# xingchensong/TouchNet

Hardware: AMD Instinct MI355X
Metric: audio+text tokens/sec/node (packed seq, full train step) + step MFU (higher is better)
Workload: dtype bf16

## Files before the change

### touchnet_amd/bin/train.py

```python
from __future__ import annotations

import os

from dataclasses import dataclass
from typing import Optional

import torch
import torch.distributed as dist

from touchnet_amd.utils.distributed import ParallelDims, dist_sum
from touchnet_amd.utils.optimizer import FusedAdamW, linear_warmup_linear_decay
from touchnet_amd.utils.train_spec import TrainSpec, get_train_spec


@dataclass
class TrainConfig:
    training_model_name: str = "llama_mi355"
    training_seed: int = 2025
    training_max_norm: float = 1.0
    training_mixed_precision_param: str = "bfloat16"
    training_mixed_precision_reduce: str = "float32"
    training_fsdp_reshard_after_forward: str = "never"
    training_tp_sequence_parallel: bool = True
    training_enable_loss_parallel: bool = False
# ... 86 lines not shown
                                enable_loss_parallel=job.training_enable_loss_parallel)
            if sharded and n == 1:
                dims = _ForceShard(dims)
            view = {"dp_shard_cp": fsdp_mesh}
            if tp > 1:
                view["tp"] = self.tp_mesh
            import dataclasses
            model = self.spec.parallelize_fn(model, _MeshView(view), dims,
                                             dataclasses.replace(job, training_dp_engine="fsdp2"))
        if sharded:
            model.to_empty(device=device)
            with torch.no_grad():
                model.post_init()
                if self.spec.additional_post_init_fn:
                    self.spec.additional_post_init_fn(model, device)
        else:
            model.to_empty(device=device)
            with torch.no_grad():
                model.post_init()
                if self.spec.additional_post_init_fn:
                    self.spec.additional_post_init_fn(model, device)
            if device.type == "cuda":
                model.to(getattr(torch, job.training_mixed_precision_param))
        if tp > 1:
            from touchnet_amd.models.tensor_parallel import reinit_tp_shards
            seq_cfg = getattr(model_config, "text_config", model_config)
            reinit_tp_shards(model, job.training_seed, getattr(seq_cfg, "initializer_range", 0.02))
        self.model = model
        self.dp_engine = None
        if flat:
            from touchnet_amd.utils.zero_dp import FlatShardedDataParallel
            self.dp_engine = FlatShardedDataParallel(model, fsdp_mesh,
                                                     reduce_dtype=getattr(torch, job.training_mixed_precision_reduce))
        if optimizer_factory is not None:
            self.optimizer = optimizer_factory(self.dp_engine.named_shards() if flat else model.parameters())
        elif flat:
            self.optimizer = FusedAdamW(self.dp_engine.named_shards(), lr=job.lr_scheduler_lr,
                                        weight_decay=job.optimizer_weight_decay, max_norm=job.training_max_norm,
                                        process_group=fsdp_mesh.get_group())
        else:
            from touchnet_amd.models.tensor_parallel import tp_param_ids
            tp_group, tp_ids = tp_param_ids([model])
            self.optimizer = FusedAdamW(model.named_parameters(), lr=job.lr_scheduler_lr,
                                        weight_decay=job.optimizer_weight_decay, max_norm=job.training_max_norm,
                                        process_group=fsdp_mesh.get_group() if sharded else None,
                                        tp_group=tp_group, tp_param_ids=tp_ids)
            want = os.environ.get("TN_PIPELINE_OPTIMIZER")
            want = job.training_pipeline_optimizer if want is None else want == "1"
            if (want and device.type == "cuda" and not sharded
                    and not any(hasattr(p, "_local_tensor") for p in model.parameters())):
                from touchnet_amd.utils.optimizer import pipeline_updates_under_forward
                pipeline_updates_under_forward(model, self.optimizer)
        self.wgrad_queue = None
        if (device.type == "cuda" and not sharded and not flat and tp == 1 and not ac and self.cp_group is None
                and self.cp_emulate is None):
            import touchnet_amd.functional as _F
            layers = [ly for m in model.modules() if hasattr(m, "deferred_wgrad_layers") for ly in m.deferred_wgrad_layers()]
            if layers and _F.DEFERRED_WGRAD:
                self.wgrad_queue = _F.DeferredWgrad(layers)
                self.wgrad_queue.enabled = False
        self.step = 0
        self.dp_cp_group = fsdp_mesh.get_group() if fsdp_mesh is not None and shard_world > 1 else None

    def next_batch(self, batch: dict) -> dict:
        out = {}
        for k, v in batch.items():
            out[k] = v.to(self.device, non_blocking=True) if isinstance(v, torch.Tensor) else v
        ns = out["num_sentence"]
        ns = ns.to(self.device, torch.float32) if isinstance(ns, torch.Tensor) else torch.tensor(
            float(ns), dtype=torch.float32, device=self.device)
        out["num_sentence"] = dist_sum(ns.reshape(1), self.dp_group) if self.dp_world > 1 else ns.reshape(1)
        if self.cp_group is not None or self.cp_emulate is not None:
            from touchnet_amd.utils.context_parallel import ContextParallel
            T = out["labels"].shape[1]
            if self.cp is None or self.cp.T != T:
                self.cp = ContextParallel(self.cp_group, T, emulate=self.cp_emulate)
            if not isinstance(out.get("attention_mask"), torch.Tensor):
                out["attention_mask"] = torch.ones(out["labels"].shape[0], T, dtype=torch.int64, device=self.device)
            if self.job.training_cp_halo_exchange:
                src = batch.get("attention_mask")
                self.cp.set_documents(src if isinstance(src, torch.Tensor) else out["attention_mask"])
            else:
                self.cp.need = None
            presharded = out.pop("audio_cp_sharded", False)
            if isinstance(out.get("audio_positions"), torch.Tensor) and not presharded:
                self._shard_audio(batch, out)
            if "labelled_rows_max" in out:
                lab = batch.get("labels")
                if "labelled_rows_max_cp" in out:
                    out["labelled_rows_max"] = int(out.pop("labelled_rows_max_cp")[self.cp.rank])
                elif isinstance(lab, torch.Tensor) and not lab.is_cuda:
                    out["labelled_rows_max"] = int((self.cp.shard(lab, dim=1) != -100).sum())
                else:
                    out.pop("labelled_rows_max")
            for k in ("input_ids", "labels", "position_ids", "sentence_lens", "input_features", "inputs_embeds"):
                if isinstance(out.get(k), torch.Tensor) and not (k == "input_features" and "audio_rows" in out):
                    out[k] = self.cp.shard(out[k], dim=1)
            out.pop("valid_rows_max", None)
            out["context_parallel"] = self.cp
        return out

    def _shard_audio(self, batch: dict, out: dict) -> None:
        host = lambda k: (batch[k] if isinstance(batch.get(k), torch.Tensor) and not batch[k].is_cuda else out[k].cpu()).numpy()
        feats = out["input_features"]
        rows_per_clip = ((feats.shape[-1] - 1) // 2 + 1) // 2
        clips, pos, rows = self.cp.shard_audio(host("audio_positions"), host("audio_output_lengths"), rows_per_clip)
        dev = lambda a: torch.from_numpy(a).to(self.device, non_blocking=True)
        clips_d = dev(clips)
        out["input_features"] = feats.index_select(0, clips_d)
        out["audio_output_lengths"] = out["audio_output_lengths"].index_select(0, clips_d)
        out["audio_positions"], out["audio_rows"] = dev(pos), dev(rows)

    def forward_loss(self, data: dict):
        data = dict(data)
        labels, ns, sl = data.pop("labels"), data.pop("num_sentence"), data.pop("sentence_lens")
        data.pop("shift_labels", None)
        if self.job.training_enable_fused_ce:
            pred = self.model(**data, labels=labels, sentence_lens=sl, num_sentence=ns,
                              ce_chunk_tokens=self.job.training_ce_chunk_tokens,
                              ce_compact=self.job.training_ce_compact_rows)
            return pred.loss, pred.loss_per_token, pred.acc
        pred = self.model(**data)
        loss, per_token = self.spec.loss_fn(pred.logits, labels, sl, ns)
        acc = self.spec.acc_fn(pred.logits, labels) if self.spec.acc_fn else None
        return loss, per_token, acc

    def train_step(self, data: dict) -> dict:
        self.optimizer.zero_grad()
        if self.dp_engine is not None:
            self.dp_engine.zero_grad()
        loss, per_token, acc = self.forward_loss(data)
        if self.wgrad_queue is not None:
            self.wgrad_queue.enabled = True
            try:
                loss.backward()
                self.wgrad_queue.flush()
            finally:
                self.wgrad_queue.enabled = False
        else:
            loss.backward()
        from touchnet_amd.models.backend import ops as _ops
        if hasattr(_ops(), "sync_wgrad_stream"):
            _ops().sync_wgrad_stream()
        if self.tp_mesh is not None:
            from touchnet_amd.models.tensor_parallel import reduce_sequence_partial_grads
            reduce_sequence_partial_grads(self.model)
        if self.dp_engine is not None:
            self.dp_engine.finish_backward()
        lr = self.job.lr_scheduler_lr * linear_warmup_linear_decay(
            self.step, self.job.lr_scheduler_warmup_steps, self.job.lr_scheduler_steps)
        grad_norm = self.optimizer.step(lr)
        if self.dp_engine is not None:
            self.dp_engine.gather_params()
        self.step += 1
        return {"loss_per_sample": loss.detach(), "loss_per_token": per_token, "acc": acc, "grad_norm": grad_norm}

    def reduce_metrics(self, loss_per_sample, loss_per_token, acc=None):
        from touchnet_amd.utils.distributed import dist_max, dist_mean, dist_min
        g = self.dp_cp_group
        ls, lt = loss_per_sample.detach(), loss_per_token.detach()
        zero = torch.zeros((), device=ls.device)
        if g is None:
            a = acc.detach() if acc is not None else zero
            return (ls, lt, lt, a, a)
        return (dist_sum(ls, g), dist_mean(lt, g), dist_max(lt, g),
                dist_mean(acc.detach(), g) if acc is not None else zero,
                dist_min(acc.detach(), g) if acc is not None else zero)

    @torch.no_grad()
    def dev_step(self, data: dict):
        return self.reduce_metrics(*self.forward_loss(data))

    @torch.no_grad()
    def dev(self, batches) -> dict:
        was_training = self.model.training
        self.model.eval()
        if getattr(self.optimizer, "wait_updates", None):
            self.optimizer.wait_updates()
        try:
            metrics = [self.dev_step(self.next_batch(b)) for b in batches]
        finally:
            self.model.train(was_training)
        if not metrics:
            return {}
        col = lambda i: torch.stack([m[i].reshape(()) for m in metrics])
        return {"global_avg_loss_per_sample": col(0).mean(), "global_avg_loss_per_token": col(1).mean(),
                "global_max_loss_per_token": col(2).max(), "global_avg_acc": col(3).mean(),
                "global_min_acc": col(4).min(), "batches": len(metrics)}
```

### touchnet_amd/csrc/gemm_kernel.h

```cpp
#pragma once

#include <stdlib.h>

#include <type_traits>
#include <utility>
#include <vector>

#include "common.h"

namespace tn {
namespace gemm {

constexpr int BM = 256, BN = 256;
constexpr int SLOT = 32768;
constexpr int LDS_BYTES = 5 * SLOT;
constexpr int NT = 512;
constexpr int MAXSEG = 3;

typedef __attribute__((address_space(3))) void* lds_ptr_t;
typedef __attribute__((ext_vector_type(2))) uint32_t u32x2_t;
typedef __attribute__((ext_vector_type(4))) uint32_t u32x4_t;

struct Seg {
  const bf16_t* A;
  const bf16_t* B;
  long long lda, ldb;
  int K;
  int pad_;
};

struct Grp {
  bf16_t* C;
  long long ldc;
  int M, N, nbm, nbn;
  int start;
  int stages;
};

struct Rec {
  Seg seg;
  Grp grp;
  bf16_t* bias_out;
};
typedef const __attribute__((address_space(4))) Rec* rec_ptr_t;
constexpr int MAXTAB = 1024;
constexpr int TABCHUNK = 32;

constexpr int EPI_PLAIN = 0, EPI_GROUPED = 1, EPI_SWIGLU_FWD = 2, EPI_SWIGLU_BWD = 3, EPI_BIASG = 4, EPI_ROPE = 5;
constexpr int EPI_GELU_FWD = 6, EPI_GELU_BWD = 7, EPI_TABLE = 8;

struct Params {
  Seg seg[MAXSEG];
  int nseg;
  int M, N;
  bf16_t* C;
  bf16_t* Ct;
  const bf16_t* bias;
  long long ldc, ldct;
  int accumulate;
  const bf16_t* addend;
  long long ldadd;
  int nbm, nbn;
  int stages;
  int splitk, kchunk;
  float* ws;
  int tile0, ntiles;
  int c_f32;
  Grp grp[MAXSEG];
  int ngrp;
  bf16_t* C2;
  bf16_t* C3;
  const bf16_t* E1;
  const bf16_t* E2;
  long long lde;
  bf16_t* bias_out;
  float* bias_ws;
  const bf16_t* rope_cos;
  const bf16_t* rope_sin;
  int rope_d;
  const Rec* table;
};

__device__ __forceinline__ int xcd_chunk(int bid, int total) {
  const int xcd = bid & 7, local = bid >> 3;
  const int q = total >> 3, r = total & 7;
  return (xcd < r ? xcd * (q + 1) : r * (q + 1) + (xcd - r) * q) + local;
}

__device__ __forceinline__ void panel_group(int vid, int nbm, int nbn, int& tm, int& tn) {
  constexpr int GM = 8;
  const int per_group = GM * nbn;
  const int g = vid / per_group, w = vid - g * per_group;
  const int gm = min(GM, nbm - g * GM);
  tm = g * GM + w % gm;
  tn = w / gm;
}

__device__ __forceinline__ void tile_of_block(int bid, int nbm, int nbn, int& tm, int& tn) {
  panel_group(xcd_chunk(bid, nbm * nbn), nbm, nbn, tm, tn);
}

typedef f32x16_t Acc[4][2];
// ... 29 lines not shown
        const int row = wave * 32 + q * 8 + (lane >> 3);
        voff[q] = row * ld2 + (((lane & 7) ^ ((row >> 1) & 7)) << 4);
      }
    } else {
#pragma unroll
      for (int q = 0; q < 4; ++q) {
        const int k = wave * 8 + q * 2 + (lane >> 5);
        const int u = lane & 31;
        const int ch = M16 ? ((u & 3) ^ (((k >> 3) & 1) << 1)) : (u & 3);
        voff[q] = k * ld2 + ((((u >> 2) ^ (k & 3)) << 6) | (ch << 4));
      }
    }
  }

  __device__ __forceinline__ void open(const bf16_t* X, long long ld, int K, int R, int origin, int wave, int lane) {
    ld2 = (int)(ld * 2);
    if constexpr (!KMAJ) {
      const long long bytes = R > origin ? (long long)(R - origin - 1) * ld2 + 2LL * K : 0LL;
      rs = __builtin_amdgcn_make_buffer_rsrc((void*)(X + (long long)origin * ld), 0, (int)min(bytes, 0x7fffffffLL),
                                             0x00020000);
      step = 128;
    } else {
      const long long bytes = ((long long)(K - 1) * ld + (R - origin)) * 2;
      rs = __builtin_amdgcn_make_buffer_rsrc((void*)(X + origin), 0, (int)min(bytes, 0x7fffffffLL), 0x00020000);
      step = 64 * ld2;
    }
    set_voff(wave, lane);
    soff = 0;
    left = (K + 63) >> 6;
  }
  __device__ __forceinline__ void kill(const void* any) {
    rs = __builtin_amdgcn_make_buffer_rsrc((void*)any, 0, 0, 0x00020000);
    soff = 0;
    step = 0;
    left = 0x7fffffff;
  }
};

template <bool KMAJ, int NB>
struct Frags {
  bf16x8_t v[NB];
  u32x2_t h[KMAJ ? NB : 1][2];
};

template <int OFF>
__device__ __forceinline__ u32x2_t ds_tr16(uint32_t addr) {
  u32x2_t r;
  asm volatile("ds_read_b64_tr_b16 %0, %1 offset:%2" : "=v"(r) : "v"(addr), "n"(OFF));
  return r;
}

template <bool AK, bool BK, bool HAS_CT, bool SPLITK = false, bool OUT_F32 = false, int EPI = EPI_PLAIN>
struct Kernel {
  static_assert(EPI == EPI_PLAIN || EPI == EPI_GROUPED || EPI == EPI_BIASG || EPI == EPI_TABLE,
                "Kernel: plain / grouped / bias-gradient epilogues (the fused ones are Kernel16's)");
  static constexpr bool MULTI = EPI == EPI_GROUPED || EPI == EPI_TABLE;
  static constexpr bool BIASG = EPI == EPI_BIASG || EPI == EPI_TABLE;
  static_assert(!MULTI || (!HAS_CT && !SPLITK), "grouped launch: whole tiles, no transposed copy");
  static_assert(!BIASG || (AK && BK && !HAS_CT), "bias gradient: weight-gradient mode");
  struct Out {
    bf16_t* C;
    long long ldc;
    int M, N;
  };
  template <bool KMAJ, int NB>
  struct Reader {
    int x[4];
    __device__ __forceinline__ Reader(int lane, int row0 ) {
      const int l31 = lane & 31, hi = lane >> 5;
      if constexpr (!KMAJ) {
        const int f = (l31 >> 1) & 7;
#pragma unroll
        for (int q = 0; q < 4; ++q) x[q] = (row0 + l31) * 128 + (((2 * q + hi) ^ f) << 4);
      } else {
        const int s4 = lane & 15, j = s4 >> 2, w = s4 & 3, half = (lane >> 4) & 1;
#pragma unroll
        for (int b = 0; b < 4; ++b)
          x[b] = (8 * hi + j) * 512 + half * 32 + w * 8 + ((((row0 >> 5) + (b < NB ? b : 0)) ^ j) << 6);
      }
    }
    template <int Q, int B>
    __device__ __forceinline__ void read(const char* smem, int sbase, Frags<KMAJ, NB>& f) const {
      if constexpr (!KMAJ) {
        f.v[B] = __builtin_bit_cast(bf16x8_t, *reinterpret_cast<const u32x4_t*>(smem + sbase + x[Q] + B * 4096));
      } else {
        const uint32_t a = (uint32_t)(size_t)(lds_ptr_t)smem + (uint32_t)(sbase + x[B]);
        f.h[B][0] = ds_tr16<(16 * Q) * 512>(a);
        f.h[B][1] = ds_tr16<(16 * Q + 4) * 512>(a);
      }
    }
  };

  static __device__ __forceinline__ void wait_frags(Frags<AK, 4>& a, Frags<BK, 2>& b) {
    if constexpr (AK && BK) {
      asm volatile("s_waitcnt lgkmcnt(0)"
                   : "+v"(a.h[0][0]), "+v"(a.h[0][1]), "+v"(a.h[1][0]), "+v"(a.h[1][1]), "+v"(a.h[2][0]), "+v"(a.h[2][1]),
                     "+v"(a.h[3][0]), "+v"(a.h[3][1]), "+v"(b.h[0][0]), "+v"(b.h[0][1]), "+v"(b.h[1][0]), "+v"(b.h[1][1]));
    } else if constexpr (AK) {
      asm volatile("s_waitcnt lgkmcnt(0)"
                   : "+v"(a.h[0][0]), "+v"(a.h[0][1]), "+v"(a.h[1][0]), "+v"(a.h[1][1]), "+v"(a.h[2][0]), "+v"(a.h[2][1]),
                     "+v"(a.h[3][0]), "+v"(a.h[3][1]));
    } else if constexpr (BK) {
      asm volatile("s_waitcnt lgkmcnt(0)" : "+v"(b.h[0][0]), "+v"(b.h[0][1]), "+v"(b.h[1][0]), "+v"(b.h[1][1]));
    }
    if constexpr (AK) {
#pragma unroll
      for (int i = 0; i < 4; ++i) {
        const u32x4_t t = {a.h[i][0].x, a.h[i][0].y, a.h[i][1].x, a.h[i][1].y};
        a.v[i] = __builtin_bit_cast(bf16x8_t, t);
      }
    }
    if constexpr (BK) {
#pragma unroll
      for (int j = 0; j < 2; ++j) {
        const u32x4_t t = {b.h[j][0].x, b.h[j][0].y, b.h[j][1].x, b.h[j][1].y};
        b.v[j] = __builtin_bit_cast(bf16x8_t, t);
      }
    }
  }

  static __device__ __forceinline__ void run(const Params& p, char* smem) { body(p, smem); }

  static __device__ __forceinline__ void body(const Params& p, char* smem) {
    const int tid = threadIdx.x;
    int lane = tid & 63;
    const int wave = __builtin_amdgcn_readfirstlane(tid >> 6);
    const int wr = wave >> 2, wc = wave & 3;

    const int bid = blockIdx.x, G = gridDim.x;
    const int tiles = p.ntiles;
    const int mine = ((SPLITK ? tiles * p.splitk : tiles) - bid + G - 1) / G;
    const rec_ptr_t tab = (rec_ptr_t)p.table;
    auto seg_of = [&](int g) {
      if constexpr (EPI == EPI_TABLE) {
        Seg s;
        s.A = tab[g].seg.A;
        s.B = tab[g].seg.B;
        s.lda = tab[g].seg.lda;
        s.ldb = tab[g].seg.ldb;
        s.K = tab[g].seg.K;
        s.pad_ = 0;
        return s;
      } else {
        return p.seg[g];
      }
    };
    auto grp_of = [&](int g) {
      if constexpr (EPI == EPI_TABLE) {
        Grp r;
        r.C = tab[g].grp.C;
        r.ldc = tab[g].grp.ldc;
        r.M = tab[g].grp.M;
        r.N = tab[g].grp.N;
        r.nbm = tab[g].grp.nbm;
        r.nbn = tab[g].grp.nbn;
        r.start = tab[g].grp.start;
        r.stages = tab[g].grp.stages;
        return r;
      } else {
        return p.grp[g];
      }
    };
    auto origin_g = [&](int k, int& m0, int& n0, int& g) {
      int tm, tn, u = bid + k * G;
      if constexpr (SPLITK) u -= (u / tiles) * tiles;
      u += p.tile0;
      g = 0;
      if constexpr (EPI == EPI_TABLE) {
        u = xcd_chunk(u, tiles);
        int hi = p.ngrp - 1;
        while (g < hi) {
          const int mid = (g + hi + 1) >> 1;
          if (tab[mid].grp.start <= u) g = mid;
          else hi = mid - 1;
        }
      } else if constexpr (EPI == EPI_GROUPED) {
        if (p.ngrp > 1 && u >= p.grp[1].start) g = 1;
        if (p.ngrp > 2 && u >= p.grp[2].start) g = 2;
      }
      if constexpr (EPI == EPI_TABLE) {
        const Grp r = grp_of(g);
        panel_group(u - r.start, r.nbm, r.nbn, tm, tn);
      } else if constexpr (EPI == EPI_GROUPED) {
        const Grp r = grp_of(g);
        tile_of_block(u - r.start, r.nbm, r.nbn, tm, tn);
      } else {
        tile_of_block(u, p.nbm, p.nbn, tm, tn);
      }
      m0 = tm * BM;
      n0 = tn * BN;
    };
    auto origin = [&](int k, int& m0, int& n0) {
      int g;
      origin_g(k, m0, n0, g);
    };
    auto split_of = [&](int k) { return (bid + k * G) / tiles; };

    Stream<AK> sA;
    Stream<BK> sB;
    int ka = 0, kb = 0;
    auto open_a = [&](int s) {
      int m0, n0;
      origin(ka, m0, n0);
      if constexpr (SPLITK) {
        const int k0 = split_of(ka) * p.kchunk * 64, klen = min(p.seg[0].K - k0, p.kchunk * 64);
        if (klen > 0) sA.open(p.seg[0].A + (AK ? (long long)k0 * p.seg[0].lda : (long long)k0), p.seg[0].lda, klen, p.M,
                              m0, wave, lane);
        else sA.kill(p.C);
        sA.left = p.kchunk;
      } else if constexpr (MULTI) {
        int g;
        origin_g(ka, m0, n0, g);
        const Seg sg = seg_of(g);
        sA.open(sg.A, sg.lda, sg.K, grp_of(g).M, m0, wave, lane);
      } else {
        sA.open(p.seg[s].A, p.seg[s].lda, p.seg[s].K, p.M, m0, wave, lane);
      }
      sA.seg = s;
    };
    auto open_b = [&](int s) {
      int m0, n0;
      origin(kb, m0, n0);
      if constexpr (SPLITK) {
        const int k0 = split_of(kb) * p.kchunk * 64, klen = min(p.seg[0].K - k0, p.kchunk * 64);
        if (klen > 0) sB.open(p.seg[0].B + (BK ? (long long)k0 * p.seg[0].ldb : (long long)k0), p.seg[0].ldb, klen, p.N,
                              n0, wave, lane);
        else sB.kill(p.C);
        sB.left = p.kchunk;
      } else if constexpr (MULTI) {
        int g;
        origin_g(kb, m0, n0, g);
        const Seg sg = seg_of(g);
        sB.open(sg.B, sg.ldb, sg.K, grp_of(g).N, n0, wave, lane);
// ... 30 lines not shown
    open_b(0);

    Reader<AK, 4> ra(lane, wr * 128);
    Reader<BK, 2> rb(lane, wc * 64);

    Acc acc;
    auto zero_acc = [&]() {
#pragma unroll
      for (int i = 0; i < 4; ++i)
#pragma unroll
        for (int j = 0; j < 2; ++j)
#pragma unroll
          for (int r = 0; r < 16; ++r) acc[i][j][r] = 0.f;
    };
    zero_acc();

    Frags<AK, 4> ae, ao;
    Frags<BK, 2> be, bo;

#define TN_PIN() __builtin_amdgcn_sched_barrier(0)
    auto read_frag = [&](auto QC, auto FC, int sa, int sb, Frags<AK, 4>& a, Frags<BK, 2>& b) {
      constexpr int Q = decltype(QC)::value, F = decltype(FC)::value;
      if constexpr (F < 2) rb.template read<Q, F>(smem, sb * SLOT, b);
      else ra.template read<Q, F - 2>(smem, sa * SLOT, a);
    };
    auto read_all = [&](auto QC, int sa, int sb, Frags<AK, 4>& a, Frags<BK, 2>& b) {
      read_frag(QC, std::integral_constant<int, 0>{}, sa, sb, a, b);
      read_frag(QC, std::integral_constant<int, 1>{}, sa, sb, a, b);
      read_frag(QC, std::integral_constant<int, 2>{}, sa, sb, a, b);
      read_frag(QC, std::integral_constant<int, 3>{}, sa, sb, a, b);
      read_frag(QC, std::integral_constant<int, 4>{}, sa, sb, a, b);
      read_frag(QC, std::integral_constant<int, 5>{}, sa, sb, a, b);
    };
    auto mma = [&](const Frags<AK, 4>& a, const Frags<BK, 2>& b, int i, int j) {
      acc[i][j] = __builtin_amdgcn_mfma_f32_32x32x16_bf16(b.v[j], a.v[i], acc[i][j], 0, 0, 0);
    };

    float bsum = 0.f;
    bool bias_on = false;
    auto bias_accum = [&](const Frags<AK, 4>& a) {
      auto add = [&](const bf16x8_t& v) {
        const u32x4_t w = __builtin_bit_cast(u32x4_t, v);
        bsum += ((__uint_as_float(w.x << 16) + __uint_as_float(w.x & 0xffff0000u)) +
                 (__uint_as_float(w.y << 16) + __uint_as_float(w.y & 0xffff0000u))) +
                ((__uint_as_float(w.z << 16) + __uint_as_float(w.z & 0xffff0000u)) +
                 (__uint_as_float(w.w << 16) + __uint_as_float(w.w & 0xffff0000u)));
      };
      if (wc == 0) add(a.v[0]);
      else if (wc == 1) add(a.v[1]);
      else if (wc == 2) add(a.v[2]);
      else add(a.v[3]);
    };

    auto quarter = [&](auto NQC, auto P0C, const Frags<AK, 4>& ca, const Frags<BK, 2>& cb, Frags<AK, 4>& na,
                       Frags<BK, 2>& nb, int nsa, int nsb, int dst_b, int dst_a) {
      constexpr int P0 = decltype(P0C)::value;
      if constexpr (BIASG) {
        if (bias_on) bias_accum(ca);
        TN_PIN();
      }
      auto step = [&](auto MC) {
        constexpr int m = decltype(MC)::value;
        mma(ca, cb, m >> 1, m & 1);
        TN_PIN();
        if constexpr (m < 6) {
          read_frag(NQC, std::integral_constant<int, m>{}, nsa, nsb, na, nb);
          TN_PIN();
        }
        constexpr int pb = P0 < 0 ? -1 : piece_at<false>(P0 + m);
        constexpr int pa = P0 < 0 ? -1 : piece_at<true>(P0 + m);
        if constexpr (pb >= 0) {
          piece_b(dst_b, pb);
          if constexpr (pb == 3) adv_b();
          TN_PIN();
        }
        if constexpr (pa >= 0) {
          piece_a(dst_a, pa);
          if constexpr (pa == 3) adv_a();
          TN_PIN();
        }
      };
      step(std::integral_constant<int, 0>{});
      step(std::integral_constant<int, 1>{});
      step(std::integral_constant<int, 2>{});
      step(std::integral_constant<int, 3>{});
      step(std::integral_constant<int, 4>{});
      step(std::integral_constant<int, 5>{});
      step(std::integral_constant<int, 6>{});
      step(std::integral_constant<int, 7>{});
    };
    auto early_pieces = [&](int dst_b, int dst_a) {
      auto one = [&](auto MC) {
        constexpr int m = decltype(MC)::value;
        constexpr int pb = piece_at<false>(m), pa = piece_at<true>(m);
        if constexpr (pb >= 0) {
          piece_b(dst_b, pb);
          if constexpr (pb == 3) adv_b();
        }
        if constexpr (pa >= 0) {
          piece_a(dst_a, pa);
          if constexpr (pa == 3) adv_a();
        }
      };
      one(std::integral_constant<int, 0>{});
      one(std::integral_constant<int, 1>{});
      one(std::integral_constant<int, 2>{});
      one(std::integral_constant<int, 3>{});
      one(std::integral_constant<int, 4>{});
      one(std::integral_constant<int, 5>{});
      one(std::integral_constant<int, 6>{});
      one(std::integral_constant<int, 7>{});
    };
    auto next = [](int s, int d) { s += d; return s >= 5 ? s - 5 : s; };
    using I0 = std::integral_constant<int, 0>;
    using I1 = std::integral_constant<int, 1>;
    using I2 = std::integral_constant<int, 2>;
    using I3 = std::integral_constant<int, 3>;
    using NONE = std::integral_constant<int, -1>;

#pragma unroll
    for (int q = 0; q < 4; ++q) piece_a(0, q);
    adv_a();
#pragma unroll
    for (int q = 0; q < 4; ++q) piece_b(1, q);
    adv_b();
#pragma unroll
    for (int q = 0; q < 4; ++q) piece_a(2, q);
    adv_a();
    early_pieces(3, 4);
    asm volatile("s_waitcnt vmcnt(%0)" ::"n"(4 + early_piece_count()) : "memory");
    __builtin_amdgcn_s_barrier();
    int sa = 0, sb = 1;
    int pa = 4, pb = 3;

    auto trip = [&](auto LASTC) {
      constexpr bool LAST = decltype(LASTC)::value;
      const int sa1 = next(sa, 2), sb1 = next(sb, 2);
      __builtin_amdgcn_s_setprio(1);
      quarter(I1{}, std::integral_constant<int, 8>{}, ae, be, ao, bo, sa, sb, pb, pa);
      wait_frags(ao, bo);
      TN_PIN();
      quarter(I2{}, std::integral_constant<int, 16>{}, ao, bo, ae, be, sa, sb, pb, pa);
      wait_frags(ae, be);
      TN_PIN();
      quarter(I3{}, std::integral_constant<int, 24>{}, ae, be, ao, bo, sa, sb, pb, pa);
      __builtin_amdgcn_s_setprio(0);
      wait_frags(ao, bo);
      __builtin_amdgcn_s_waitcnt(0xc07f);
      asm volatile("s_waitcnt vmcnt(4)" ::: "memory");
      __builtin_amdgcn_s_barrier();
      __builtin_amdgcn_s_setprio(1);
      if constexpr (!LAST) {
        quarter(I0{}, I0{}, ao, bo, ae, be, sa1, sb1, sa, sb);
        __builtin_amdgcn_s_setprio(0);
        wait_frags(ae, be);
        TN_PIN();
      } else {
        if constexpr (BIASG) {
          if (bias_on) bias_accum(ao);
        }
#pragma unroll
        for (int m = 0; m < 8; ++m) mma(ao, bo, m >> 1, m & 1);
        __builtin_amdgcn_s_setprio(0);
      }
      pb = sa;
      pa = sb;
      sa = sa1;
      sb = sb1;
    };

    const int np_all = SPLITK ? p.kchunk : p.stages;
    for (int kc = 0; kc < mine; ++kc) {
      int np = np_all;
      if constexpr (BIASG) {
        int m0_, n0_, g_;
        origin_g(kc, m0_, n0_, g_);
        bias_on = n0_ == 0;
        if constexpr (EPI == EPI_TABLE) bias_on = bias_on && tab[g_].bias_out != nullptr;
        bsum = 0.f;
      }
      if constexpr (MULTI) {
        int m0_, n0_, g_;
        origin_g(kc, m0_, n0_, g_);
        np = grp_of(g_).stages;
      }
      read_all(I0{}, sa, sb, ae, be);
      wait_frags(ae, be);
      TN_PIN();
      for (int t = 1; t < np; ++t) trip(std::false_type{});
      trip(std::true_type{});
      int m0, n0, grp;
      origin_g(kc, m0, n0, grp);
      if constexpr (BIASG) {
        if (bias_on) {
          const float tot = bsum + __shfl_xor(bsum, 32, 64);
          const int m = m0 + wr * 128 + wc * 32 + (lane & 31);
          if (lane < 32) {
            if constexpr (SPLITK) {
              p.bias_ws[(long long)split_of(kc) * (p.nbm * BM) + m] = tot;
            } else if constexpr (EPI == EPI_TABLE) {
              if (m < tab[grp].grp.M) tab[grp].bias_out[m] = f2bf(tot);
            } else if (m < p.M) {
              p.bias_out[m] = f2bf(tot);
            }
          }
        }
      }
      if constexpr (SPLITK) {
        const int u = bid + kc * G, sp = u / tiles;
        epilogue_ws(p, acc, sp * tiles + (u - sp * tiles), wr * 128, wc * 64, lane);
      } else if constexpr (OUT_F32) {
        if constexpr (MULTI) {
          const Grp r = grp_of(grp);
          const Out o = {r.C, r.ldc, r.M, r.N};
          epilogue_f32(p, o, acc, m0 + wr * 128, n0 + wc * 64, lane);
        } else {
          const Out o = {p.C, p.ldc, p.M, p.N};
          epilogue_f32(p, o, acc, m0 + wr * 128, n0 + wc * 64, lane);
        }
      } else if constexpr (MULTI) {
        const Grp r = grp_of(grp);
        const Out o = {r.C, r.ldc, r.M, r.N};
        epilogue(p, o, acc, smem + (wave < 4 ? pb : pa) * SLOT + (wave & 3) * 8192, m0 + wr * 128, n0 + wc * 64, lane);
      } else {
        const Out o = {p.C, p.ldc, p.M, p.N};
        epilogue(p, o, acc, smem + (wave < 4 ? pb : pa) * SLOT + (wave & 3) * 8192, m0 + wr * 128, n0 + wc * 64, lane);
      }
      zero_acc();
      __builtin_amdgcn_s_waitcnt(0xc07f);
      __builtin_amdgcn_s_barrier();
      asm volatile("" : "+v"(lane));
      ra = Reader<AK, 4>(lane, wr * 128);
      rb = Reader<BK, 2>(lane, wc * 64);
      sA.set_voff(wave, lane);
      sB.set_voff(wave, lane);
      early_pieces(pb, pa);
    }
  }

  static __device__ __forceinline__ void epilogue_f32(const Params& p, const Out& o, Acc& acc, int wm0, int wn0, int lane) {
    const int l31 = lane & 31, hi = lane >> 5;
    float* C = reinterpret_cast<float*>(o.C);
    const bool add = p.accumulate != 0;
#pragma unroll
    for (int i = 0; i < 4; ++i) {
      const int m = wm0 + i * 32 + l31;
#pragma unroll
      for (int j = 0; j < 2; ++j)
#pragma unroll
        for (int g = 0; g < 4; ++g) {
          const int n = wn0 + j * 32 + 8 * g + 4 * hi;
          if (m < o.M && n < o.N) {
            f32x4_t* dst = reinterpret_cast<f32x4_t*>(C + (long long)m * o.ldc + n);
// ... 121 lines not shown
```

### touchnet_amd/csrc/gemm_table.hip

```cpp
#include "gemm_host.h"

namespace tn {
namespace gemm {

struct RecChunk {
  Rec r[TABCHUNK];
};
static_assert(sizeof(Rec) % 8 == 0 && sizeof(RecChunk) <= 3072, "a chunk of records fits the kernel-argument segment");
constexpr int REC_WORDS = (int)(sizeof(Rec) / 8);

__global__ __launch_bounds__(TABCHUNK * REC_WORDS) void table_upload_kernel(const RecChunk c, Rec* dst, int n) {
  const int t = threadIdx.x;
  if (t < n * REC_WORDS)
    reinterpret_cast<unsigned long long*>(dst)[t] = reinterpret_cast<const unsigned long long*>(&c)[t];
}

}
}

extern "C" {

long long tn_gemm_grouped_table_bytes(int n) { return n < 1 || n > MAXTAB ? -1 : (long long)n * (long long)sizeof(Rec); }

int tn_gemm_bf16_grouped_table(const void* const* A, const void* const* B, const long long* lda, const long long* ldb,
                               const int* K, void* const* C, const long long* ldc, const int* M, const int* N,
                               void* const* bias_grad, int n, int accumulate, int c_f32, void* table, long long table_bytes,
                               void* stream) {
  if (n < 1 || n > MAXTAB) return TN_EINVAL;
  if (table == nullptr || !aligned(15, table) || table_bytes < tn_gemm_grouped_table_bytes(n)) return TN_EINVAL;
  std::vector<RecChunk> chunks((n + TABCHUNK - 1) / TABCHUNK);
  long long total = 0;
  for (int g = 0; g < n; ++g) {
    Rec& r = chunks[g / TABCHUNK].r[g % TABCHUNK];
    if (total > 0x7fffffff) return TN_EINVAL;
    if (!grouped_product(A[g], B[g], lda[g], ldb[g], K[g], C[g], ldc[g], M[g], N[g], c_f32, (int)total, r.seg, r.grp))
      return TN_EINVAL;
    r.bias_out = bias_grad != nullptr ? (bf16_t*)bias_grad[g] : nullptr;
    if (!aligned(1, r.bias_out)) return TN_EINVAL;
    total += (long long)r.grp.nbm * r.grp.nbn;
  }
  if (total > 0x7fffffff) return TN_EINVAL;
  hipStream_t st = (hipStream_t)stream;
  for (int c = 0; c * TABCHUNK < n; ++c)
    hipLaunchKernelGGL(table_upload_kernel, dim3(1), dim3(TABCHUNK * REC_WORDS), 0, st, chunks[c],
                       (Rec*)table + c * TABCHUNK, min(TABCHUNK, n - c * TABCHUNK));
  Params p;
  clear_params(p);
  p.table = (const Rec*)table;
  p.ngrp = n;
  p.accumulate = accumulate;
  p.c_f32 = c_f32;
  p.ntiles = (int)total;
  if (c_f32)
    hipLaunchKernelGGL((gemm_kernel<true, true, false, false, true, EPI_TABLE>), grid_for(p.ntiles), dim3(NT), 0, st, p);
  else
    hipLaunchKernelGGL((gemm_kernel<true, true, false, false, false, EPI_TABLE>), grid_for(p.ntiles), dim3(NT), 0, st, p);
  TN_LAUNCH_CHECK();
  return TN_OK;
}

}
```

### touchnet_amd/functional.py

```python
from __future__ import annotations

import ctypes
import math
import os
import weakref
from dataclasses import dataclass
from typing import Optional

import torch

from . import _C
from . import library as L

_cur = _C.stream
_p = _C.ptr


def _c(t: torch.Tensor) -> torch.Tensor:
    return t if t.is_contiguous() else t.contiguous()


def rms_norm(x, weight, eps, residual=None):
    y, h, _ = L.rmsnorm_fwd(x, residual, weight, float(eps))
    return (y, h) if residual is not None else y
# ... 689 lines not shown


def _beside(inputs, fn, written=()):
    side = WGRAD_STREAM
    if side is None:
        return fn()
    global WGRAD_MAIN
    main = torch.cuda.current_stream()
    WGRAD_MAIN = main
    side.wait_stream(main)
    with torch.cuda.stream(side):
        out = fn()
    for t in inputs:
        t.record_stream(side)
    wait = False
    for t in written:
        if t is not None:
            t.record_stream(side)
            wait = True
    outs = out if isinstance(out, (list, tuple)) else (out,)
    for t in outs:
        if isinstance(t, torch.Tensor):
            t.record_stream(main)
            wait = wait or WGRAD_RETURNS_NEED_SYNC
    if wait:
        main.wait_stream(side)
    return out


GRAD_SINKS = {}


def _live(table, w):
    ref = table.get(id(w))
    return ref() if ref is not None else None


def _sink_of(w):
    sink = _live(GRAD_SINKS, w)
    return sink if sink is not None and sink.owns(w) else None


DEFERRED_WGRAD = True
DEFERRED_WGRAD_FLUSH_LAYERS = 11
WGRAD_QUEUES = {}


def _queue_of(w):
    return _live(WGRAD_QUEUES, w)


class DeferredWgrad:

    def __init__(self, layers, flush_layers: int = DEFERRED_WGRAD_FLUSH_LAYERS):
        if flush_layers < 1:
            raise ValueError("DeferredWgrad: flush_layers >= 1")
        self.flush_layers = flush_layers
        self.launch = gemm_grouped_table_wgrad
        self.enabled = True
        self._owned = {}
        self._items = []
        self._waiting = set()
        self._layers = set()
        self.flushes = 0
        for li, layer in enumerate(layers):
            for w, b in layer:
                self._owned[id(w)] = (w, b, li)
                WGRAD_QUEUES[id(w)] = weakref.ref(self)

    def __len__(self):
        return len(self._items)

    def close(self):
        if self._items:
            raise _C.KernelError("DeferredWgrad.close: the queue is not empty")
        for k in self._owned:
            ref = WGRAD_QUEUES.get(k)
            if ref is not None and ref() is self:
                del WGRAD_QUEUES[k]
        self._owned = {}

    def push(self, w, dy, x2, with_bias: bool) -> bool:
        own = self._owned.get(id(w))
        if not self.enabled or own is None or own[0] is not w:
            return False
        _, bias, layer = own
        if id(w) in self._waiting:
            raise _C.KernelError("DeferredWgrad: a weight was queued twice without a flush in between "
                                 "(two backward passes through one layer: flush between them)")
        ok = (_wgrad_own(dy, x2, queued=True) and w.dtype == torch.bfloat16 and tuple(w.shape) == (dy.shape[1], x2.shape[1])
              and (not with_bias or (bias is not None and bias.dtype == torch.bfloat16))
              and (w.grad is None or (w.grad.dtype == torch.bfloat16 and w.grad.is_contiguous()
                                      and (w.grad.is_meta or w.grad.data_ptr() % 16 == 0))))
        if not ok:
            return False
        if layer not in self._layers and len(self._layers) >= self.flush_layers:
            self.flush()
        self._items.append((w, dy, x2, bias if with_bias else None, torch.cuda.current_stream() if dy.is_cuda else None))
        self._waiting.add(id(w))
        self._layers.add(layer)
        return True

    def flush(self) -> None:
        items, self._items = self._items, []
        self._waiting.clear()
        self._layers.clear()
        if not items:
            return
        self.flushes += 1
        cur = torch.cuda.current_stream() if items[0][1].is_cuda else None
        for w, dy, x2, _, st in items:
            if st is not None and st != cur:
                cur.wait_stream(st)
                dy.record_stream(cur)
                x2.record_stream(cur)
        parts = {acc: [it for it in items if (it[0].grad is not None) == acc] for acc in (False, True)}
        for acc, part in parts.items():
            for i in range(0, len(part), GROUPED_TABLE_MAX):
                chunk = part[i:i + GROUPED_TABLE_MAX]
                outs = [w.grad if acc else torch.empty(w.shape, dtype=torch.bfloat16, device=dy.device)
                        for w, dy, _, _, _ in chunk]
                bgs = [torch.empty(dy.shape[1], dtype=torch.bfloat16, device=dy.device) if b is not None else None
                       for _, dy, _, b, _ in chunk]
                self.launch([(dy, x2) for _, dy, x2, _, _ in chunk], outs=outs, accumulate=acc, bias_grads=bgs)
                for (w, _, _, b, _), o, bg in zip(chunk, outs, bgs):
                    if not acc:
                        w.grad = o
                    if b is not None:
                        if b.grad is None:
                            b.grad = bg
                        else:
                            b.grad.add_(bg)


def _queue_wgrad(w, dy, x2, with_bias: bool) -> bool:
    if not DEFERRED_WGRAD or WGRAD_STREAM is not None:
        return False
    q = _queue_of(w)
    return q is not None and _sink_of(w) is None and q.push(w, dy, x2, with_bias)


def _route_wgrad(w, dy, x2, want_bias: bool = False):
    ride = bool(want_bias and BIAS_IN_WGRAD)
    if _queue_wgrad(w, dy, x2, ride):
        return None, None, True
    if not _wgrad_own(dy, x2):
        return None, None, False
    sink = _sink_of(w)
    db = torch.empty(dy.shape[1], dtype=torch.bfloat16, device=dy.device) if ride else None

    def launch():
        if sink is None:
            return gemm([(dy, x2)], True, True, bias_grad=db)
# ... 786 lines not shown
```

### touchnet_amd/models/llama/modeling_llama.py

```python
from __future__ import annotations

import os
from types import SimpleNamespace
from typing import Optional

import torch
import torch.nn as nn

from ..backend import ops
from .configuration import DecoderConfig


class RMSNorm(nn.Module):
    def __init__(self, hidden_size, eps):
        super().__init__()
        self.weight = nn.Parameter(torch.ones(hidden_size))
        self.variance_epsilon = eps

    def forward(self, x, residual=None):
        return ops().rms_norm(x, self.weight, self.variance_epsilon, residual=residual)


class RotaryEmbedding(nn.Module):
    def __init__(self, config: DecoderConfig):
# ... 75 lines not shown
SKIP_PAD_ROWS = os.environ.get("TN_SKIP_PAD_ROWS", "1") != "0"


LAST_LAYER_LABELLED_ROWS = os.environ.get("TN_LAST_LAYER_LABELLED_ROWS", "1") != "0"


class MLP(nn.Module):
    def __init__(self, config: DecoderConfig):
        super().__init__()
        H, I = config.hidden_size, config.intermediate_size
        self.gate_proj = nn.Linear(H, I, bias=False)
        self.up_proj = nn.Linear(H, I, bias=False)
        self.down_proj = nn.Linear(I, H, bias=False)

    def forward(self, x, norm_src=None):
        kw = {"norm_src": norm_src} if norm_src is not None else {}
        return ops().swiglu_mlp(x, self.gate_proj.weight, self.up_proj.weight, self.down_proj.weight, **kw)


class DecoderLayer(nn.Module):
    def __init__(self, config: DecoderConfig):
        super().__init__()
        self.self_attn = Attention(config)
        self.mlp = MLP(config)
        self.input_layernorm = RMSNorm(config.hidden_size, config.rms_norm_eps)
        self.post_attention_layernorm = RMSNorm(config.hidden_size, config.rms_norm_eps)

    def forward(self, delta, residual, cos, sin, mask, keep_rows=None, kv_out=None):
        sac = getattr(self, "_tn_recompute_rows", False) and torch.is_grad_enabled()
        if residual is None:
            residual = delta
            x = self.input_layernorm(delta)
        else:
            x, residual = self.input_layernorm(delta, residual)
        src = ops().norm_source(residual, self.input_layernorm.weight, self.input_layernorm.variance_epsilon) if sac else None
        a = (self.self_attn(x, cos, sin, mask, keep_rows, norm_src=src) if kv_out is None
             else self.self_attn(x, cos, sin, mask, keep_rows, norm_src=src, kv_out=kv_out))
        if keep_rows is not None:
            residual = residual.reshape(-1, residual.shape[-1]).index_select(0, keep_rows)[None]
        x, residual = self.post_attention_layernorm(a, residual)
        src = (ops().norm_source(residual, self.post_attention_layernorm.weight, self.post_attention_layernorm.variance_epsilon)
               if sac else None)
        return self.mlp(x, norm_src=src), residual


class DecoderModel(nn.Module):
    def __init__(self, config: DecoderConfig):
        super().__init__()
        self.config = config
        self.embed_tokens = nn.Embedding(config.vocab_size, config.hidden_size)
        self.layers = nn.ModuleList([DecoderLayer(config) for _ in range(config.num_hidden_layers)])
        self.norm = RMSNorm(config.hidden_size, config.rms_norm_eps)
        self.rotary_emb = RotaryEmbedding(config)

    @staticmethod
    def _drop_pad_rows(inputs_embeds, position_ids, doc, keep_rows, valid_rows_max):
        B, T, H = inputs_embeds.shape
        Mc = min((int(valid_rows_max) + 255) // 256 * 256, B * T)
        if Mc + 256 > B * T:
            return None
        flat = doc.reshape(-1)
        is_pad = flat <= 0
        order = torch.sort(is_pad.to(torch.int8), stable=True).indices
        rows = order[:Mc]
        overflow = (~is_pad).sum() > Mc
        uniq = doc.to(torch.int64) + (torch.arange(B, device=doc.device, dtype=torch.int64) * (T + 1))[:, None]
        doc_c = torch.where(is_pad, torch.zeros_like(flat, dtype=torch.int64), uniq.reshape(-1)).index_select(0, rows)[None]
        emb_c = inputs_embeds.reshape(B * T, H).index_select(0, rows)[None]
        pos_c = position_ids.reshape(-1).index_select(0, rows)[None]
        if keep_rows is not None:
            inv = torch.zeros(B * T, dtype=torch.int64, device=rows.device)
            inv[rows] = torch.arange(Mc, device=rows.device)
            keep_rows = inv.index_select(0, keep_rows)
        return emb_c, pos_c, doc_c, keep_rows, rows, overflow

    def forward(self, input_ids=None, inputs_embeds=None, position_ids=None, attention_mask=None,
                context_parallel=None, keep_rows=None, valid_rows_max=None, kv_out=None):
        if inputs_embeds is None:
            inputs_embeds = self.embed_tokens(input_ids)
        B, T, _ = inputs_embeds.shape
        if position_ids is None:
            position_ids = torch.arange(T, device=inputs_embeds.device).expand(B, T)
        sp = getattr(self, "_tn_sp", None)
        dropped = None
        if (SKIP_PAD_ROWS and valid_rows_max is not None and context_parallel is None and sp is None and kv_out is None
                and isinstance(attention_mask, torch.Tensor) and attention_mask.dim() == 2
                and not attention_mask.dtype.is_floating_point):
            dropped = self._drop_pad_rows(inputs_embeds, position_ids, attention_mask, keep_rows, valid_rows_max)
        if dropped is not None:
            inputs_embeds, position_ids, attention_mask, keep_rows, kept, overflow = dropped
            full_shape = (B, T)
            B, T = 1, inputs_embeds.shape[1]
        cos, sin = self.rotary_emb(position_ids, inputs_embeds.dtype)
        mask = attention_mask
        if mask is None:
            mask = ops().causal_mask(B, T, inputs_embeds.device)
        elif isinstance(mask, torch.Tensor):
            mask = ops().build_packed_mask(mask)
        if context_parallel is not None:
            mask.cp = context_parallel
        if sp is not None and keep_rows is not None:
            raise RuntimeError("keep_rows is not available under sequence parallelism")
        if sp is not None and kv_out is not None:
            raise RuntimeError("kv_out is not available under sequence parallelism")
        kw = {} if kv_out is None else {"kv_out": kv_out}
        delta, residual = (inputs_embeds if sp is None else sp.scatter(inputs_embeds)), None
# ... 98 lines not shown
```

Before: 23600.

## Batch attention QKV weight-gradient GEMMs per layer into one grouped table launch

Adds a second deferred weight-gradient queue for each decoder layer's q/k/v projections. The queue collects the three wgrad GEMMs, including their bias gradients, and flushes them as one grouped table launch as soon as the layer's set is complete. Only whole-tile, non-split-K shapes are accepted. The table GEMM kernel gains a variant with no bias epilogue, and bias accumulation becomes a per-tile compile-time branch, so launches without bias skip that work. The aim is fewer small kernel launches and better GPU fill during backward, at the cost of extra kernel instantiations and queue bookkeeping.

```diff
diff --git a/touchnet_amd/bin/train.py b/touchnet_amd/bin/train.py
--- a/touchnet_amd/bin/train.py
+++ b/touchnet_amd/bin/train.py
@@ -162,6 +162,7 @@
                 from touchnet_amd.utils.optimizer import pipeline_updates_under_forward
                 pipeline_updates_under_forward(model, self.optimizer)
         self.wgrad_queue = None
+        self.attn_wgrad_queue = None
         if (device.type == "cuda" and not sharded and not flat and tp == 1 and not ac and self.cp_group is None
                 and self.cp_emulate is None):
             import touchnet_amd.functional as _F
@@ -169,6 +170,10 @@
             if layers and _F.DEFERRED_WGRAD:
                 self.wgrad_queue = _F.DeferredWgrad(layers)
                 self.wgrad_queue.enabled = False
+            layers = [ly for m in model.modules() if hasattr(m, "attention_wgrad_layers") for ly in m.attention_wgrad_layers()]
+            if layers and _F.DEFERRED_WGRAD:
+                self.attn_wgrad_queue = _F.DeferredWgrad(layers, flush_layers=1, whole_only=True, flush_when_complete=True)
+                self.attn_wgrad_queue.enabled = False
         self.step = 0
         self.dp_cp_group = fsdp_mesh.get_group() if fsdp_mesh is not None and shard_world > 1 else None
 
@@ -235,20 +240,24 @@
         acc = self.spec.acc_fn(pred.logits, labels) if self.spec.acc_fn else None
         return loss, per_token, acc
 
+    def backward(self, loss) -> None:
+        queues = [q for q in (self.attn_wgrad_queue, self.wgrad_queue) if q is not None]
+        for q in queues:
+            q.enabled = True
+        try:
+            loss.backward()
+            for q in queues:
+                q.flush()
+        finally:
+            for q in queues:
+                q.enabled = False
+
     def train_step(self, data: dict) -> dict:
         self.optimizer.zero_grad()
         if self.dp_engine is not None:
             self.dp_engine.zero_grad()
         loss, per_token, acc = self.forward_loss(data)
-        if self.wgrad_queue is not None:
-            self.wgrad_queue.enabled = True
-            try:
-                loss.backward()
-                self.wgrad_queue.flush()
-            finally:
-                self.wgrad_queue.enabled = False
-        else:
-            loss.backward()
+        self.backward(loss)
         from touchnet_amd.models.backend import ops as _ops
         if hasattr(_ops(), "sync_wgrad_stream"):
             _ops().sync_wgrad_stream()
diff --git a/touchnet_amd/csrc/gemm_kernel.h b/touchnet_amd/csrc/gemm_kernel.h
--- a/touchnet_amd/csrc/gemm_kernel.h
+++ b/touchnet_amd/csrc/gemm_kernel.h
@@ -47,7 +47,7 @@
 constexpr int TABCHUNK = 32;
 
 constexpr int EPI_PLAIN = 0, EPI_GROUPED = 1, EPI_SWIGLU_FWD = 2, EPI_SWIGLU_BWD = 3, EPI_BIASG = 4, EPI_ROPE = 5;
-constexpr int EPI_GELU_FWD = 6, EPI_GELU_BWD = 7, EPI_TABLE = 8;
+constexpr int EPI_GELU_FWD = 6, EPI_GELU_BWD = 7, EPI_TABLE = 8, EPI_TABLE_PLAIN = 9;
 
 struct Params {
   Seg seg[MAXSEG];
@@ -183,10 +183,12 @@
 
 template <bool AK, bool BK, bool HAS_CT, bool SPLITK = false, bool OUT_F32 = false, int EPI = EPI_PLAIN>
 struct Kernel {
-  static_assert(EPI == EPI_PLAIN || EPI == EPI_GROUPED || EPI == EPI_BIASG || EPI == EPI_TABLE,
+  static_assert(EPI == EPI_PLAIN || EPI == EPI_GROUPED || EPI == EPI_BIASG || EPI == EPI_TABLE || EPI == EPI_TABLE_PLAIN,
                 "Kernel: plain / grouped / bias-gradient epilogues (the fused ones are Kernel16's)");
-  static constexpr bool MULTI = EPI == EPI_GROUPED || EPI == EPI_TABLE;
+  static constexpr bool TABLE = EPI == EPI_TABLE || EPI == EPI_TABLE_PLAIN;
+  static constexpr bool MULTI = EPI == EPI_GROUPED || TABLE;
   static constexpr bool BIASG = EPI == EPI_BIASG || EPI == EPI_TABLE;
+  static constexpr bool BIAS_PER_TILE = EPI == EPI_TABLE;
   static_assert(!MULTI || (!HAS_CT && !SPLITK), "grouped launch: whole tiles, no transposed copy");
   static_assert(!BIASG || (AK && BK && !HAS_CT), "bias gradient: weight-gradient mode");
   struct Out {
@@ -263,7 +265,7 @@
     const int mine = ((SPLITK ? tiles * p.splitk : tiles) - bid + G - 1) / G;
     const rec_ptr_t tab = (rec_ptr_t)p.table;
     auto seg_of = [&](int g) {
-      if constexpr (EPI == EPI_TABLE) {
+      if constexpr (TABLE) {
         Seg s;
         s.A = tab[g].seg.A;
         s.B = tab[g].seg.B;
@@ -277,7 +279,7 @@
       }
     };
     auto grp_of = [&](int g) {
-      if constexpr (EPI == EPI_TABLE) {
+      if constexpr (TABLE) {
         Grp r;
         r.C = tab[g].grp.C;
         r.ldc = tab[g].grp.ldc;
@@ -297,7 +299,7 @@
       if constexpr (SPLITK) u -= (u / tiles) * tiles;
       u += p.tile0;
       g = 0;
-      if constexpr (EPI == EPI_TABLE) {
+      if constexpr (TABLE) {
         u = xcd_chunk(u, tiles);
         int hi = p.ngrp - 1;
         while (g < hi) {
@@ -309,7 +311,7 @@
         if (p.ngrp > 1 && u >= p.grp[1].start) g = 1;
         if (p.ngrp > 2 && u >= p.grp[2].start) g = 2;
       }
-      if constexpr (EPI == EPI_TABLE) {
+      if constexpr (TABLE) {
         const Grp r = grp_of(g);
         panel_group(u - r.start, r.nbm, r.nbn, tm, tn);
       } else if constexpr (EPI == EPI_GROUPED) {
@@ -446,11 +448,11 @@
       else add(a.v[3]);
     };
 
-    auto quarter = [&](auto NQC, auto P0C, const Frags<AK, 4>& ca, const Frags<BK, 2>& cb, Frags<AK, 4>& na,
+    auto quarter = [&](auto BC, auto NQC, auto P0C, const Frags<AK, 4>& ca, const Frags<BK, 2>& cb, Frags<AK, 4>& na,
                        Frags<BK, 2>& nb, int nsa, int nsb, int dst_b, int dst_a) {
       constexpr int P0 = decltype(P0C)::value;
-      if constexpr (BIASG) {
-        if (bias_on) bias_accum(ca);
+      if constexpr (decltype(BC)::value) {
+        if (BIAS_PER_TILE || bias_on) bias_accum(ca);
         TN_PIN();
       }
       auto step = [&](auto MC) {
@@ -527,17 +529,17 @@
     int sa = 0, sb = 1;
     int pa = 4, pb = 3;
 
-    auto trip = [&](auto LASTC) {
+    auto trip = [&](auto LASTC, auto BC) {
       constexpr bool LAST = decltype(LASTC)::value;
       const int sa1 = next(sa, 2), sb1 = next(sb, 2);
       __builtin_amdgcn_s_setprio(1);
-      quarter(I1{}, std::integral_constant<int, 8>{}, ae, be, ao, bo, sa, sb, pb, pa);
+      quarter(BC, I1{}, std::integral_constant<int, 8>{}, ae, be, ao, bo, sa, sb, pb, pa);
       wait_frags(ao, bo);
       TN_PIN();
-      quarter(I2{}, std::integral_constant<int, 16>{}, ao, bo, ae, be, sa, sb, pb, pa);
+      quarter(BC, I2{}, std::integral_constant<int, 16>{}, ao, bo, ae, be, sa, sb, pb, pa);
       wait_frags(ae, be);
       TN_PIN();
-      quarter(I3{}, std::integral_constant<int, 24>{}, ae, be, ao, bo, sa, sb, pb, pa);
+      quarter(BC, I3{}, std::integral_constant<int, 24>{}, ae, be, ao, bo, sa, sb, pb, pa);
       __builtin_amdgcn_s_setprio(0);
       wait_frags(ao, bo);
       __builtin_amdgcn_s_waitcnt(0xc07f);
@@ -545,13 +547,13 @@
       __builtin_amdgcn_s_barrier();
       __builtin_amdgcn_s_setprio(1);
       if constexpr (!LAST) {
-        quarter(I0{}, I0{}, ao, bo, ae, be, sa1, sb1, sa, sb);
+        quarter(BC, I0{}, I0{}, ao, bo, ae, be, sa1, sb1, sa, sb);
         __builtin_amdgcn_s_setprio(0);
         wait_frags(ae, be);
         TN_PIN();
       } else {
-        if constexpr (BIASG) {
-          if (bias_on) bias_accum(ao);
+        if constexpr (decltype(BC)::value) {
+          if (BIAS_PER_TILE || bias_on) bias_accum(ao);
         }
 #pragma unroll
         for (int m = 0; m < 8; ++m) mma(ao, bo, m >> 1, m & 1);
@@ -570,7 +572,7 @@
         int m0_, n0_, g_;
         origin_g(kc, m0_, n0_, g_);
         bias_on = n0_ == 0;
-        if constexpr (EPI == EPI_TABLE) bias_on = bias_on && tab[g_].bias_out != nullptr;
+        if constexpr (TABLE) bias_on = bias_on && tab[g_].bias_out != nullptr;
         bsum = 0.f;
       }
       if constexpr (MULTI) {
@@ -581,8 +583,18 @@
       read_all(I0{}, sa, sb, ae, be);
       wait_frags(ae, be);
       TN_PIN();
-      for (int t = 1; t < np; ++t) trip(std::false_type{});
-      trip(std::true_type{});
+      if constexpr (BIAS_PER_TILE) {
+        if (bias_on) {
+          for (int t = 1; t < np; ++t) trip(std::false_type{}, std::true_type{});
+          trip(std::true_type{}, std::true_type{});
+        } else {
+          for (int t = 1; t < np; ++t) trip(std::false_type{}, std::false_type{});
+          trip(std::true_type{}, std::false_type{});
+        }
+      } else {
+        for (int t = 1; t < np; ++t) trip(std::false_type{}, std::integral_constant<bool, BIASG>{});
+        trip(std::true_type{}, std::integral_constant<bool, BIASG>{});
+      }
       int m0, n0, grp;
       origin_g(kc, m0, n0, grp);
       if constexpr (BIASG) {
@@ -592,7 +604,7 @@
           if (lane < 32) {
             if constexpr (SPLITK) {
               p.bias_ws[(long long)split_of(kc) * (p.nbm * BM) + m] = tot;
-            } else if constexpr (EPI == EPI_TABLE) {
+            } else if constexpr (TABLE) {
               if (m < tab[grp].grp.M) tab[grp].bias_out[m] = f2bf(tot);
             } else if (m < p.M) {
               p.bias_out[m] = f2bf(tot);
diff --git a/touchnet_amd/csrc/gemm_table.hip b/touchnet_amd/csrc/gemm_table.hip
--- a/touchnet_amd/csrc/gemm_table.hip
+++ b/touchnet_amd/csrc/gemm_table.hip
@@ -30,6 +30,7 @@
   if (table == nullptr || !aligned(15, table) || table_bytes < tn_gemm_grouped_table_bytes(n)) return TN_EINVAL;
   std::vector<RecChunk> chunks((n + TABCHUNK - 1) / TABCHUNK);
   long long total = 0;
+  bool any_bias = false;
   for (int g = 0; g < n; ++g) {
     Rec& r = chunks[g / TABCHUNK].r[g % TABCHUNK];
     if (total > 0x7fffffff) return TN_EINVAL;
@@ -37,6 +38,7 @@
       return TN_EINVAL;
     r.bias_out = bias_grad != nullptr ? (bf16_t*)bias_grad[g] : nullptr;
     if (!aligned(1, r.bias_out)) return TN_EINVAL;
+    any_bias = any_bias || r.bias_out != nullptr;
     total += (long long)r.grp.nbm * r.grp.nbn;
   }
   if (total > 0x7fffffff) return TN_EINVAL;
@@ -51,10 +53,14 @@
   p.accumulate = accumulate;
   p.c_f32 = c_f32;
   p.ntiles = (int)total;
-  if (c_f32)
+  if (c_f32 && any_bias)
     hipLaunchKernelGGL((gemm_kernel<true, true, false, false, true, EPI_TABLE>), grid_for(p.ntiles), dim3(NT), 0, st, p);
+  else if (c_f32)
+    hipLaunchKernelGGL((gemm_kernel<true, true, false, false, true, EPI_TABLE_PLAIN>), grid_for(p.ntiles), dim3(NT), 0, st, p);
+  else if (any_bias)
+    hipLaunchKernelGGL((gemm_kernel<true, true, false, false, false, EPI_TABLE>), grid_for(p.ntiles), dim3(NT), 0, st, p);
   else
-    hipLaunchKernelGGL((gemm_kernel<true, true, false, false, false, EPI_TABLE>), grid_for(p.ntiles), dim3(NT), 0, st, p);
+    hipLaunchKernelGGL((gemm_kernel<true, true, false, false, false, EPI_TABLE_PLAIN>), grid_for(p.ntiles), dim3(NT), 0, st, p);
   TN_LAUNCH_CHECK();
   return TN_OK;
 }
diff --git a/touchnet_amd/functional.py b/touchnet_amd/functional.py
--- a/touchnet_amd/functional.py
+++ b/touchnet_amd/functional.py
@@ -765,10 +765,14 @@
 
 class DeferredWgrad:
 
-    def __init__(self, layers, flush_layers: int = DEFERRED_WGRAD_FLUSH_LAYERS):
+    def __init__(self, layers, flush_layers: int = DEFERRED_WGRAD_FLUSH_LAYERS, whole_only: bool = False,
+                 flush_when_complete: bool = False):
         if flush_layers < 1:
             raise ValueError("DeferredWgrad: flush_layers >= 1")
         self.flush_layers = flush_layers
+        self.whole_only = whole_only
+        self.flush_when_complete = flush_when_complete
+        self._layer_size = [len(layer) for layer in layers]
         self.launch = gemm_grouped_table_wgrad
         self.enabled = True
         self._owned = {}
@@ -801,6 +805,10 @@
         if id(w) in self._waiting:
             raise _C.KernelError("DeferredWgrad: a weight was queued twice without a flush in between "
                                  "(two backward passes through one layer: flush between them)")
+        if self.whole_only:
+            n, k, m = dy.shape[1], x2.shape[1], dy.shape[0]
+            if not _own(n, k, (m,), True, True) or (SPLIT_K and split_k(n, k, m, True, True) > 1):
+                return False
         ok = (_wgrad_own(dy, x2, queued=True) and w.dtype == torch.bfloat16 and tuple(w.shape) == (dy.shape[1], x2.shape[1])
               and (not with_bias or (bias is not None and bias.dtype == torch.bfloat16))
               and (w.grad is None or (w.grad.dtype == torch.bfloat16 and w.grad.is_contiguous()
@@ -812,6 +820,9 @@
         self._items.append((w, dy, x2, bias if with_bias else None, torch.cuda.current_stream() if dy.is_cuda else None))
         self._waiting.add(id(w))
         self._layers.add(layer)
+        if (self.flush_when_complete and len(self._layers) >= self.flush_layers
+                and len(self._items) == sum(self._layer_size[li] for li in self._layers)):
+            self.flush()
         return True
 
     def flush(self) -> None:
diff --git a/touchnet_amd/models/llama/modeling_llama.py b/touchnet_amd/models/llama/modeling_llama.py
--- a/touchnet_amd/models/llama/modeling_llama.py
+++ b/touchnet_amd/models/llama/modeling_llama.py
@@ -151,6 +151,10 @@
         self.layers = nn.ModuleList([DecoderLayer(config) for _ in range(config.num_hidden_layers)])
         self.norm = RMSNorm(config.hidden_size, config.rms_norm_eps)
         self.rotary_emb = RotaryEmbedding(config)
+
+    def attention_wgrad_layers(self):
+        return [[(lin.weight, lin.bias) for lin in (l.self_attn.q_proj, l.self_attn.k_proj, l.self_attn.v_proj)]
+                for l in self.layers]
 
     @staticmethod
     def _drop_pad_rows(inputs_embeds, position_ids, doc, keep_rows, valid_rows_max):
```

Result: no change. 23650, median of 5 (+0.2%).
